# ViktorNfa/bluerov2_dynamics

Hardware: AMD Instinct MI355X
Metric: rk4_rollout_steps_per_s (higher is better)
Workload: dtype f64; 1 GPU; BASELINE config 2: 65536 trajectories/GPU x 5000 RK4 steps, thruster model, dt=0.02, iid U(-1,1) commands (splitmix64 stream 0x5EED), layout tpb, all states stored; trajectories_per_gpu=65536, horizon=5000, parallelism=1 x independent shards, no collective

## Files before the change

bluerov2_dynamics_amd/csrc/brov2_fast.h:

```cpp
#pragma once
#include "brov2_device.h"

namespace brov {

struct FastParams {
    double E[12];
    double da[6], db[6];
    double G[5];
    double lc[4][3];
    double ld[4];
    double Tm[6][8];
    double minv[6];
    double poly[5];
    double A1[9], b1[3];
    double A4[9], b4[3];
    double Ob[9];
    double al4[3];
    double Aw4[9], bw4[3];
    double g1[3];
    double XY[4];
    double cur[3];
    int has_current;
    int has_xy;
    int tm_dense;
// ... 8 lines not shown
    static constexpr bool RESIDENT = RES;
    double E[12], db[6];
    double da[6], G[5], ld[4], al4[3];
};
typedef HotConstsT<false> HotConsts;
typedef HotConstsT<true> HotConstsResident;

#ifndef BROV_CLAMP_BRANCH
#define BROV_CLAMP_BRANCH 1
#endif
#ifndef BROV_PSI_FRAME
#define BROV_PSI_FRAME 1
#endif
#define BROV_PIN_V(x) asm volatile("" : "+v"(x))
#define BROV_PIN_S(x) asm volatile("" : "+s"(x))
#define BROV_SC(h, p, f) (HC::RESIDENT ? (h).f : (p)->f)

template <bool RES>
__device__ __forceinline__ void load_hot(CFP pp, HotConstsT<RES>& h) {
    const auto& p = *pp;
#pragma unroll
    for (int i = 0; i < 12; ++i) { h.E[i] = p.E[i]; BROV_PIN_V(h.E[i]); }
#pragma unroll
    for (int i = 0; i < 6; ++i) { h.db[i] = p.db[i]; BROV_PIN_V(h.db[i]); }
    if constexpr (RES) {
#pragma unroll
        for (int i = 0; i < 6; ++i) { h.da[i] = p.da[i]; BROV_PIN_S(h.da[i]); }
#pragma unroll
        for (int i = 0; i < 5; ++i) { h.G[i] = p.G[i]; BROV_PIN_S(h.G[i]); }
#pragma unroll
        for (int i = 0; i < 4; ++i) { h.ld[i] = p.ld[i]; BROV_PIN_S(h.ld[i]); }
#pragma unroll
        for (int i = 0; i < 3; ++i) { h.al4[i] = p.al4[i]; BROV_PIN_S(h.al4[i]); }
    }
}

__device__ __forceinline__ CFP relaunder(CFP p) {
    asm volatile("" : "+s"(p));
    return p;
}

__device__ __forceinline__ void sincos_fast(double x, double& s, double& c, const double2* __restrict__ qt) {
    const double kf = rint(x * 6.36619772367581382433e-01);
    double r = fma(-kf, 1.57079632673412561417e+00, x);
    r = fma(-kf, 6.07710050630396597660e-11, r);
    r = fma(-kf, 2.02226624879595063154e-21, r);
    const int q = (int)kf;
    const double z = r * r;
    double ps = fma(z, 1.58969099521155010221e-10, -2.50507602534068634195e-08);
    ps = fma(z, ps, 2.75573137070700676789e-06);
    ps = fma(z, ps, -1.98412698298579493134e-04);
    ps = fma(z, ps, 8.33333333332248946124e-03);
    ps = fma(z, ps, -1.66666666666666324348e-01);
    const double sr = fma(z * r, ps, r);
    double pc = fma(z, -1.13596475577881948265e-11, 2.08757232129817482790e-09);
    pc = fma(z, pc, -2.75573143513906633035e-07);
    pc = fma(z, pc, 2.48015872894767294178e-05);
    pc = fma(z, pc, -1.38888888888741095749e-03);
    pc = fma(z, pc, 4.16666666666666019037e-02);
    const double cr = fma(z * z, pc, fma(-0.5, z, 1.0));
    const double2 t = qt[q & 3];
    s = fma(cr, t.y, sr * t.x);
    c = fma(-sr, t.y, cr * t.x);
}

__device__ __forceinline__ void init_quadrant_table(double2* qt) {
    if (threadIdx.x < 4) {
        const int q = threadIdx.x;
        qt[q] = make_double2(q == 0 ? 1.0 : (q == 2 ? -1.0 : 0.0), q == 1 ? 1.0 : (q == 3 ? -1.0 : 0.0));
    }
}

struct Trig { double sphi, cphi, sth, cth, spsi, cpsi; };

__device__ __forceinline__ void trig_full(const double* ang, Trig& t, const double2* __restrict__ qt) {
    sincos_fast(ang[0], t.sphi, t.cphi, qt);
    sincos_fast(ang[1], t.sth, t.cth, qt);
    sincos_fast(ang[2], t.spsi, t.cpsi, qt);
}

template <bool SHORT = false>
__device__ __forceinline__ void trig_delta(const Trig& b, const double d[3], Trig& t, double* dpsi = nullptr) {
    double dd[3] = {d[0], d[1], d[2]};
    int k = 0;
    const double m = fmax(fmax(fabs(d[0]), fabs(d[1])), fabs(d[2]));
    if (!(m <= (SHORT ? 0.0625 : 0.125))) {
        int e;
        (void)frexp(m, &e);
        k = e + (SHORT ? 4 : 3);
        double sc = ldexp(1.0, -k);
        if (!(m < 0x1p37)) { sc = __builtin_nan(""); k = 0; }
#pragma unroll
        for (int i = 0; i < 3; ++i) dd[i] *= sc;
    }
    double sd[3], cm[3];
#pragma unroll
    for (int i = 0; i < 3; ++i) {
        const double z = dd[i] * dd[i];
        double ps, pc;
        if constexpr (SHORT) {
            ps = fma(z, -1.98412698298579493134e-04, 8.33333333332248946124e-03);
            pc = fma(z, 2.48015872894767294178e-05, -1.38888888888741095749e-03);
        } else {
            ps = fma(z, 2.75573137070700676789e-06, -1.98412698298579493134e-04);
            ps = fma(z, ps, 8.33333333332248946124e-03);
            pc = fma(z, -2.75573143513906633035e-07, 2.48015872894767294178e-05);
            pc = fma(z, pc, -1.38888888888741095749e-03);
        }
        ps = fma(z, ps, -1.66666666666666324348e-01);
        sd[i] = fma(z * dd[i], ps, dd[i]);
        pc = fma(z, pc, 4.16666666666666019037e-02);
        pc = fma(z, pc, -0.5);
        cm[i] = z * pc;
    }
    for (int j = 0; j < k; ++j) {
#pragma unroll
        for (int i = 0; i < 3; ++i) {
            const double t2 = sd[i] + sd[i];
            const double s2 = fma(t2, cm[i], t2);
            cm[i] = -(t2 * sd[i]);
            sd[i] = s2;
        }
    }
    t.sphi = fma(b.cphi, sd[0], fma(b.sphi, cm[0], b.sphi)); t.cphi = fma(-b.sphi, sd[0], fma(b.cphi, cm[0], b.cphi));
    t.sth = fma(b.cth, sd[1], fma(b.sth, cm[1], b.sth));     t.cth = fma(-b.sth, sd[1], fma(b.cth, cm[1], b.cth));
    t.spsi = fma(b.cpsi, sd[2], fma(b.spsi, cm[2], b.spsi)); t.cpsi = fma(-b.spsi, sd[2], fma(b.cpsi, cm[2], b.cpsi));
    if (dpsi) { dpsi[0] = sd[2]; dpsi[1] = cm[2]; }
}

#ifndef BROV_TRIG_SHORT
#define BROV_TRIG_SHORT 1
#endif
__device__ __forceinline__ double recip_fast(double x) {
    double y = __builtin_amdgcn_rcp(x);
    double e = fma(-x, y, 1.0);
    y = fma(y, e, y);
    e = fma(-x, y, 1.0);
    return fma(y, e, y);
}

template <bool GENERIC, class HC>
__device__ __forceinline__ void nu_dot_fast(const HC& h, CFP p, const double R[9], const double nu[6],
                                            const double a[6], double sth, double ctsp, double ctcp, double out[6]) {
    const double u = nu[0], v = nu[1], w = nu[2], pp = nu[3], q = nu[4], r = nu[5];
    double nr0 = u, nr1 = v, nr2 = w;
    if (GENERIC && p->has_current) {
        nr0 -= fma(R[6], p->cur[2], fma(R[3], p->cur[1], R[0] * p->cur[0]));
        nr1 -= fma(R[7], p->cur[2], fma(R[4], p->cur[1], R[1] * p->cur[0]));
        nr2 -= fma(R[8], p->cur[2], fma(R[5], p->cur[1], R[2] * p->cur[0]));
    }
    double o0 = fma(-h.E[0], w * q, a[0]);  o0 = fma(h.E[1], v * r, o0);
    double o1 = fma(-h.E[2], u * r, a[1]);  o1 = fma(h.E[3], w * pp, o1);
    double o2 = fma(-h.E[4], v * pp, a[2]); o2 = fma(h.E[5], u * q, o2);
    double o3 = fma(-h.E[6], v * w, a[3]);  o3 = fma(-h.E[7], q * r, o3);
    double o4 = fma(-h.E[8], u * w, a[4]);  o4 = fma(-h.E[9], pp * r, o4);
    double o5 = fma(-h.E[10], u * v, a[5]); o5 = fma(-h.E[11], pp * q, o5);
    o0 = fma(-fma(h.db[0], fabs(nr0), BROV_SC(h, p, da[0])), nr0, o0);
    o1 = fma(-fma(h.db[1], fabs(nr1), BROV_SC(h, p, da[1])), nr1, o1);
    o2 = fma(-fma(h.db[2], fabs(nr2), BROV_SC(h, p, da[2])), nr2, o2);
    o3 = fma(-fma(h.db[3], fabs(pp), BROV_SC(h, p, da[3])), pp, o3);
    o4 = fma(-fma(h.db[4], fabs(q), BROV_SC(h, p, da[4])), q, o4);
    o5 = fma(-fma(h.db[5], fabs(r), BROV_SC(h, p, da[5])), r, o5);
    o0 = fma(-BROV_SC(h, p, G[0]), sth, o0);
    o1 = fma(BROV_SC(h, p, G[1]), ctsp, o1);
    o2 = fma(BROV_SC(h, p, G[2]), ctcp, o2);
    o3 = fma(BROV_SC(h, p, G[3]), ctsp, o3);
    o4 = fma(BROV_SC(h, p, G[4]), sth, o4);
    if (GENERIC && p->has_xy) {
        o3 = fma(-p->XY[0], ctcp, o3);
        o4 = fma(p->XY[1], ctcp, o4);
        o5 = fma(-p->XY[2], ctsp, o5);
        o5 = fma(-p->XY[3], sth, o5);
    }
    out[0] = o0; out[1] = o1; out[2] = o2; out[3] = o3; out[4] = o4; out[5] = o5;
}

template <bool GENERIC, class HC, bool PFRAME = false>
__device__ __forceinline__ void rhs_fast_euler(const HC& h, CFP p, const double x[12], const double a[6], double xd[12], const Trig& tg) {
    const double sphi = tg.sphi, cphi = tg.cphi, sth = tg.sth, cth = tg.cth, spsi = tg.spsi, cpsi = tg.cpsi;
    const double* nu = x + 6;
    const double ctsp = cth * sphi, ctcp = cth * cphi;
    if constexpr (GENERIC) {
        double R[9];
        const double ss = sth * sphi, sc = sth * cphi;
        R[0] = cpsi * cth; R[1] = fma(cpsi, ss, -(spsi * cphi)); R[2] = fma(cpsi, sc, spsi * sphi);
        R[3] = spsi * cth; R[4] = fma(spsi, ss, cpsi * cphi);    R[5] = fma(spsi, sc, -(cpsi * sphi));
        R[6] = -sth;       R[7] = ctsp;                          R[8] = ctcp;
        nu_dot_fast<true>(h, p, R, nu, a, sth, ctsp, ctcp, xd + 6);
#pragma unroll
        for (int i = 0; i < 3; ++i) xd[i] = fma(R[3 * i + 2], nu[2], fma(R[3 * i + 1], nu[1], R[3 * i] * nu[0]));
    } else {
        nu_dot_fast<false>(h, p, nullptr, nu, a, sth, ctsp, ctcp, xd + 6);
        const double y1 = fma(cphi, nu[1], -(sphi * nu[2])), z1 = fma(sphi, nu[1], cphi * nu[2]);
        const double x2 = fma(cth, nu[0], sth * z1), z2 = fma(cth, z1, -(sth * nu[0]));
        if constexpr (PFRAME) { xd[0] = x2; xd[1] = y1; }
        else {
            xd[0] = fma(cpsi, x2, -(spsi * y1));
            xd[1] = fma(spsi, x2, cpsi * y1);
        }
        xd[2] = z2;
    }
    double cc = cth;
#if BROV_CLAMP_BRANCH
    if (__builtin_amdgcn_ballot_w64(fabs(cc) < 1e-7) != 0) {
// ... 115 lines not shown
        }
    }
    __device__ __forceinline__ void obs_advance1(CFP p, const double acmd[6]) {
        const double c0 = p->al4[0], c1 = p->al4[1], c2 = p->al4[2], g0 = p->g1[0], g1 = p->g1[1], g2 = p->g1[2];
#pragma unroll
        for (int k = 0; k < 6; ++k) {
            const double a0 = z[k][0], a1 = z[k][1], a2 = z[k][2];
            z[k][0] = fma(g0, acmd[k], a1);
            z[k][1] = fma(g1, acmd[k], a2);
            z[k][2] = fma(c2, a2, fma(c1, a1, fma(c0, a0, g2 * acmd[k])));
        }
    }
    __device__ __forceinline__ void advance(const double __attribute__((address_space(4)))* A, const double __attribute__((address_space(4)))* b, const double acmd[6]) {
#pragma unroll
        for (int k = 0; k < 6; ++k) {
            const double a0 = z[k][0], a1 = z[k][1], a2 = z[k][2];
            const double q0 = fma(A[1], a1, fma(A[0], a0, b[0] * acmd[k]));
            const double q1 = fma(A[4], a1, fma(A[3], a0, b[1] * acmd[k]));
            const double q2 = fma(A[7], a1, fma(A[6], a0, b[2] * acmd[k]));
            double n0 = a0, n1 = a1, n2 = a2;
            asm("v_fma_f64 %0, %1, %2, %3" : "+v"(n0) : "s"(A[2]), "v"(a2), "v"(q0), "v"(q1), "v"(q2));
            asm("v_fma_f64 %0, %1, %2, %3" : "+v"(n1) : "s"(A[5]), "v"(a2), "v"(q1), "v"(q0), "v"(q2));
            asm("v_fma_f64 %0, %1, %0, %2" : "+v"(n2) : "s"(A[8]), "v"(q2), "v"(n0), "v"(n1));
            z[k][0] = n0; z[k][1] = n1; z[k][2] = n2;
        }
    }
};

__device__ __forceinline__ void advance_thrusters(const double __attribute__((address_space(4)))* A, const double __attribute__((address_space(4)))* b, const double fcmd[8], double X[8][3]) {
#pragma unroll
    for (int i = 0; i < 8; ++i) {
        const double a0 = X[i][0], a1 = X[i][1], a2 = X[i][2];
        X[i][0] = fma(A[2], a2, fma(A[1], a1, fma(A[0], a0, b[0] * fcmd[i])));
        X[i][1] = fma(A[5], a2, fma(A[4], a1, fma(A[3], a0, b[1] * fcmd[i])));
        X[i][2] = fma(A[8], a2, fma(A[7], a1, fma(A[6], a0, b[2] * fcmd[i])));
    }
}

template <int MODEL, bool SPARSE>
__device__ __forceinline__ void command_accel(CFP p, const double* u, double fcmd[8], double acmd[6]) {
    if constexpr (MODEL == MODEL_THRUSTER_EULER) {
#pragma unroll
        for (int i = 0; i < 8; ++i) {
            const double V = u[i], V2 = V * V;
            double hh = fma(V2, p->poly[4], p->poly[3]);
            hh = fma(V2, hh, p->poly[2]);
            hh = fma(V2, hh, p->poly[1]);
            hh = fma(V2, hh, p->poly[0]);
            fcmd[i] = V * hh;
        }
        if constexpr (SPARSE) {
#pragma unroll
            for (int k = 0; k < 6; ++k) {
                const int i0 = (k == 2) ? 4 : 0, i1 = (k == 3 || k == 4) ? 8 : (k == 2 ? 8 : 4);
                double a = p->Tm[k][i0] * fcmd[i0];
#pragma unroll
                for (int i = i0 + 1; i < i1; ++i) a = fma(p->Tm[k][i], fcmd[i], a);
                acmd[k] = a;
            }
        } else {
#pragma unroll
            for (int k = 0; k < 6; ++k) {
                double a = p->Tm[k][0] * fcmd[0];
#pragma unroll
                for (int i = 1; i < 8; ++i) a = fma(p->Tm[k][i], fcmd[i], a);
                acmd[k] = a;
            }
        }
    } else if constexpr (model_is_di(MODEL)) {
        constexpr int NU = Dims<MODEL>::NU;
#pragma unroll
        for (int k = 0; k < 6; ++k) {
            double a = p->Tm[k][0] * u[0];
#pragma unroll
            for (int i = 1; i < NU; ++i) a = fma(p->Tm[k][i], u[i], a);
            acmd[k] = a;
        }
    } else {
#pragma unroll
        for (int k = 0; k < 6; ++k) acmd[k] = p->minv[k] * u[k];
    }
}

template <int MODEL, int INTEG, bool GENERIC, class HC, class AccelFn>
__device__ __forceinline__ void integrate_fast(const HC& h, CFP p, double dt, double* x, AccelFn&& accel,
                                               const double2* qt, Trig* carry, bool refresh) {
    constexpr int NX = Dims<MODEL>::NX;
    constexpr bool ANG = !model_is_quat(MODEL);
    double a[6];
    Trig tb, ts;
    const bool CARRY = ANG && carry != nullptr;
    if constexpr (ANG) {
        if (!CARRY || refresh) trig_full(x + 3, tb, qt);
        else tb = *carry;
    }
    double dang[3];
    if constexpr (INTEG == INTEG_EULER) {
        double k[NX];
        accel(1, a);
        rhs_fast<MODEL, GENERIC>(h, p, x, a, k, tb);
        if (CARRY) {
#pragma unroll
            for (int i = 0; i < NX; ++i) {
                if (i >= 3 && i < 6) { dang[i - 3] = dt * k[i]; x[i] += dang[i - 3]; }
                else x[i] = fma(dt, k[i], x[i]);
            }
        } else {
#pragma unroll
            for (int i = 0; i < NX; ++i) x[i] = fma(dt, k[i], x[i]);
        }
    } else {
        double k[NX], xn[NX], xs[NX], dl[3];
        const double h2 = 0.5 * dt, h6 = dt / 6.0, h3 = dt / 3.0;
        constexpr bool PSIF = BROV_PSI_FRAME && ANG && !GENERIC && !model_is_di(MODEL);
        double dps[2] = {0.0, 0.0};
        auto stage_state = [&](double c, auto HALF) {
#pragma unroll
            for (int i = 0; i < NX; ++i) {
                if (ANG && i >= 3 && i < 6) dl[i - 3] = c * k[i];
                else xs[i] = fma(c, k[i], x[i]);
            }
            if constexpr (ANG) trig_delta<BROV_TRIG_SHORT && decltype(HALF)::value>(tb, dl, ts, PSIF ? dps : nullptr);
        };
        auto add_turned = [&](double w) {
            const double r0 = fma(dps[1], k[0], fma(-dps[0], k[1], k[0])), r1 = fma(dps[0], k[0], fma(dps[1], k[1], k[1]));
            xn[0] = fma(w, r0, xn[0]);
            xn[1] = fma(w, r1, xn[1]);
        };
        accel(1, a);
        rhs_fast<MODEL, GENERIC, HC, PSIF>(h, p, x, a, k, tb);
#pragma unroll
        for (int i = 0; i < NX; ++i) xn[i] = ((CARRY && i >= 3 && i < 6) || (PSIF && i < 2)) ? h6 * k[i] : fma(h6, k[i], x[i]);
        stage_state(h2, std::true_type{});
        accel(2, a);
        rhs_fast<MODEL, GENERIC, HC, PSIF>(h, p, xs, a, k, ts);
#pragma unroll
        for (int i = PSIF ? 2 : 0; i < NX; ++i) xn[i] = fma(h3, k[i], xn[i]);
        if constexpr (PSIF) add_turned(h3);
        stage_state(h2, std::true_type{});
        accel(3, a);
        rhs_fast<MODEL, GENERIC, HC, PSIF>(h, p, xs, a, k, ts);
#pragma unroll
        for (int i = PSIF ? 2 : 0; i < NX; ++i) xn[i] = fma(h3, k[i], xn[i]);
        if constexpr (PSIF) add_turned(h3);
        stage_state(dt, std::false_type{});
        accel(4, a);
        rhs_fast<MODEL, GENERIC, HC, PSIF>(h, p, xs, a, k, ts);
        if constexpr (PSIF) {
            add_turned(h6);
            x[0] = fma(tb.cpsi, xn[0], fma(-tb.spsi, xn[1], x[0]));
            x[1] = fma(tb.spsi, xn[0], fma(tb.cpsi, xn[1], x[1]));
        }
        if (CARRY) {
#pragma unroll
            for (int i = PSIF ? 2 : 0; i < NX; ++i) {
                if (i >= 3 && i < 6) { dang[i - 3] = fma(h6, k[i], xn[i]); x[i] += dang[i - 3]; }
                else x[i] = fma(h6, k[i], xn[i]);
            }
        } else {
#pragma unroll
            for (int i = PSIF ? 2 : 0; i < NX; ++i) x[i] = fma(h6, k[i], xn[i]);
        }
    }
    if constexpr (ANG) { if (CARRY) trig_delta(tb, dang, *carry); }
    if constexpr (model_is_quat(MODEL)) quat_normalize(x + 3);
}

template <int INTEG, int LAGMODE, bool TRACK, bool GENERIC>
__device__ __forceinline__ void lag_step_advance(CFP pl, LagZ& lz, const double fcmd[8], const double acmd[6], double X[8][3]) {
    constexpr bool OBS = !GENERIC;
    if constexpr (INTEG == INTEG_RK4 && LAGMODE == 0) {
        if constexpr (OBS) lz.advance(pl->Aw4, pl->bw4, acmd); else lz.advance(pl->A4, pl->b4, acmd);
        if constexpr (TRACK) advance_thrusters(pl->A4, pl->b4, fcmd, X);
    } else {
        if constexpr (OBS) lz.obs_advance1(pl, acmd); else lz.advance(pl->A1, pl->b1, acmd);
        if constexpr (TRACK) advance_thrusters(pl->A1, pl->b1, fcmd, X);
    }
}
template <int LAGMODE, bool GENERIC, class HC>
__device__ __forceinline__ void lag_stage_accel(const HC& h, CFP p, const LagZ& lz, int s, const double acmd[6], double a[6]) {
    const int se = LAGMODE == 0 ? s : 1;
    if constexpr (!GENERIC) lz.obs_accel_after(h, p, se, acmd, a); else lz.accel_after(p, se, acmd, a);
}

template <int MODEL, int INTEG, int LAGMODE, bool TRACK, bool GENERIC, class HC>
__device__ __forceinline__ void step_fast(const HC& h, CFP p0, double dt, double* x, const double* u,
                                          LagZ& lz, double X[8][3], const double2* qt, Trig* carry = nullptr, bool refresh = true) {
    constexpr bool THR = (MODEL == MODEL_THRUSTER_EULER);
    CFP p = relaunder(p0);
    double fcmd[8], acmd[6];
    if constexpr (MODEL == MODEL_DI_WRENCH_QUAT) quat_normalize(x + 3);
    command_accel<MODEL, !GENERIC>(p, u, fcmd, acmd);
    integrate_fast<MODEL, INTEG, GENERIC>(h, p, dt, x, [&](int s, double* a) {
        if constexpr (THR) lag_stage_accel<LAGMODE, GENERIC>(h, p, lz, s, acmd, a);
        else {
#pragma unroll
            for (int k = 0; k < 6; ++k) a[k] = acmd[k];
        }
    }, qt, carry, refresh);
    if constexpr (THR) lag_step_advance<INTEG, LAGMODE, TRACK, GENERIC>(relaunder(p0), lz, fcmd, acmd, X);
}

}
```

bluerov2_dynamics_amd/csrc/rollout.hip:

```cpp
#include "brov2_device.h"
#include "brov2_fast.h"
#include "brov2_kernels.h"

namespace brov {

constexpr int TRIG_REFRESH = 64;

#if BROV_CLOCK_STAMPS
__device__ unsigned long long g_clock_stamps[4096][4];
extern "C" __attribute__((visibility("default"))) int brov_debug_clock_stamps(unsigned long long* host, int nblocks) {
    return (int)hipMemcpyFromSymbol(host, HIP_SYMBOL(g_clock_stamps), sizeof(unsigned long long) * 4 * nblocks, 0, hipMemcpyDeviceToHost);
}
#endif

template <int N>
__device__ __forceinline__ void load_row(const double* __restrict__ src, double* r) {
    if constexpr (N % 2 == 0) {
        const double2* s2 = reinterpret_cast<const double2*>(src);
#pragma unroll
        for (int i = 0; i < N / 2; ++i) { double2 v = s2[i]; r[2 * i] = v.x; r[2 * i + 1] = v.y; }
    } else {
#pragma unroll
        for (int i = 0; i < N; ++i) r[i] = src[i];
    }
}
template <int N>
__device__ __forceinline__ void store_row(double* __restrict__ dst, const double* r) {
    if constexpr (N % 2 == 0) {
        double2* d2 = reinterpret_cast<double2*>(dst);
#pragma unroll
        for (int i = 0; i < N / 2; ++i) d2[i] = make_double2(r[2 * i], r[2 * i + 1]);
    } else {
#pragma unroll
        for (int i = 0; i < N; ++i) dst[i] = r[i];
    }
}
template <int N>
__device__ __forceinline__ void load_soa(const double* __restrict__ src, int64_t ld, double* r) {
#pragma unroll
    for (int i = 0; i < N; ++i) r[i] = src[i * ld];
}
template <int N>
__device__ __forceinline__ void store_soa(double* __restrict__ dst, int64_t ld, const double* r) {
#pragma unroll
    for (int i = 0; i < N; ++i) dst[i * ld] = r[i];
}
template <int N>
__device__ __forceinline__ void load_pairs(const double* __restrict__ p, int64_t ld2, double* r) {
#pragma unroll
    for (int i = 0; i < (N + 1) / 2; ++i) {
        typedef double v2d __attribute__((ext_vector_type(2)));
        const v2d w = __builtin_nontemporal_load(reinterpret_cast<const v2d*>(p + i * ld2));
        const double2 v = make_double2(w[0], w[1]);
        r[2 * i] = v.x;
        if (2 * i + 1 < N) r[2 * i + 1] = v.y;
    }
}
template <int N>
__device__ __forceinline__ void store_pairs(double* __restrict__ p, int64_t ld2, const double* r) {
#pragma unroll
    for (int i = 0; i < (N + 1) / 2; ++i) {
        typedef double v2d __attribute__((ext_vector_type(2)));
        v2d w; w[0] = r[2 * i]; w[1] = (2 * i + 1 < N) ? r[2 * i + 1] : 0.0;
        __builtin_nontemporal_store(w, reinterpret_cast<v2d*>(p + i * ld2));
    }
}

template <int MODEL, int INTEG, int LAGMODE>
__device__ __forceinline__ void integrate_step(const DevParams& p, double dt, double* x, const double* u, LagBank& lag) {
    constexpr int NX = Dims<MODEL>::NX;
    constexpr bool THR = (MODEL == MODEL_THRUSTER_EULER);
    double fcmd[8], F[8], tau[6];
    if constexpr (THR) {
#pragma unroll
        for (int i = 0; i < 8; ++i) fcmd[i] = thrust_poly(p, u[i]);
    } else {
#pragma unroll
        for (int i = 0; i < 6; ++i) tau[i] = u[i];
    }
    if constexpr (INTEG == INTEG_EULER) {
        double k[NX];
        if constexpr (THR) { lag.forces_after(p, 1, fcmd, F); allocate(p, F, tau); }
        rhs_state<MODEL>(p, x, tau, k);
#pragma unroll
        for (int i = 0; i < NX; ++i) x[i] = fma(dt, k[i], x[i]);
        if constexpr (THR) lag.advance(p, 1, fcmd);
    } else {
        double k[NX], acc[NX], xs[NX];
        const double h2 = 0.5 * dt;
        if constexpr (THR) { lag.forces_after(p, 1, fcmd, F); allocate(p, F, tau); }
        rhs_state<MODEL>(p, x, tau, k);
#pragma unroll
        for (int i = 0; i < NX; ++i) { acc[i] = k[i]; xs[i] = fma(h2, k[i], x[i]); }
        if constexpr (THR && LAGMODE == 0) { lag.forces_after(p, 2, fcmd, F); allocate(p, F, tau); }
// ... 84 lines not shown
    load_row<NX>(X0 + b * NX, x);
    LagZ lz;
    double Xl[8][3];
    if constexpr (MODEL == MODEL_THRUSTER_EULER) {
        if constexpr (TRACK) {
            load_row<24>(lag_io + b * 24, &Xl[0][0]);
            lz.from_thrusters(p, Xl);
        } else {
            lz.zero();
        }
        if constexpr (!GENERIC) lz.to_observer(p);
    }
    const int64_t rows = traj ? T / stride + 1 : 0;
    double* tp = nullptr;
    int64_t tstep = 0;
    constexpr int NXP = (NX + 1) / 2, NUP = (NU + 1) / 2;
    if (traj) {
        if constexpr (LAYOUT == LAYOUT_BTU) { tp = traj + b * rows * NX; tstep = NX; }
        else if constexpr (LAYOUT == LAYOUT_TUB) { tp = traj + b; tstep = (int64_t)NX * B; }
        else { tp = traj + 2 * b; tstep = (int64_t)NXP * 2 * B; }
    }
    auto store_state = [&]() {
        if constexpr (LAYOUT == LAYOUT_BTU) store_row<NX>(tp, x);
        else if constexpr (LAYOUT == LAYOUT_TUB) store_soa<NX>(tp, B, x);
        else store_pairs<NX>(tp, 2 * B, x);
        tp += tstep;
    };
    const double* up;
    int64_t ustep;
    if constexpr (LAYOUT == LAYOUT_BTU) { up = U + b * T * NU; ustep = NU; }
    else if constexpr (LAYOUT == LAYOUT_TUB) { up = U + b; ustep = (int64_t)NU * B; }
    else { up = U + 2 * b; ustep = (int64_t)NUP * 2 * B; }

    double un[NU];
    if (T > 0) {
        if constexpr (LAYOUT == LAYOUT_BTU) load_row<NU>(up, un);
        else if constexpr (LAYOUT == LAYOUT_TUB) load_soa<NU>(up, B, un);
        else load_pairs<NU>(up, 2 * B, un);
    }
    if (traj) store_state();
    int64_t countdown = stride;
    Trig tcarry;
#if BROV_CLOCK_STAMPS
    const unsigned long long st0 = __builtin_amdgcn_s_memtime(), sr0 = __builtin_amdgcn_s_memrealtime();
#endif
    for (int64_t t = 0; t < T; ++t) {
        double u[NU];
#pragma unroll
        for (int i = 0; i < NU; ++i) u[i] = un[i];
        up += (t + 1 < T) ? ustep : 0;
        {
            if constexpr (LAYOUT == LAYOUT_BTU) load_row<NU>(up, un);
            else if constexpr (LAYOUT == LAYOUT_TUB) load_soa<NU>(up, B, un);
            else load_pairs<NU>(up, 2 * B, un);
        }
        step_fast<MODEL, INTEG, LAGMODE, TRACK, GENERIC>(h, p, dt, x, u, lz, Xl, qt, &tcarry, (t & (TRIG_REFRESH - 1)) == 0);
        if (traj && --countdown == 0) {
            countdown = stride;
            store_state();
        }
    }
#if BROV_CLOCK_STAMPS
    if (threadIdx.x == 0 && blockIdx.x < 4096) {
        g_clock_stamps[blockIdx.x][0] = st0; g_clock_stamps[blockIdx.x][1] = sr0;
        g_clock_stamps[blockIdx.x][2] = __builtin_amdgcn_s_memtime(); g_clock_stamps[blockIdx.x][3] = __builtin_amdgcn_s_memrealtime();
    }
#endif
    if (XT) store_row<NX>(XT + b * NX, x);
    if constexpr (MODEL == MODEL_THRUSTER_EULER && TRACK) store_row<24>(lag_io + b * 24, &Xl[0][0]);
}

#ifndef BROV_PAIR_EXP
#define BROV_PAIR_EXP 0
#endif
#ifndef BROV_PAIR_RING
#define BROV_PAIR_RING 2
#endif
#ifndef BROV_PAIR_STAGE
#define BROV_PAIR_STAGE 1
#endif
#ifndef BROV_PAIR_PRIO
#define BROV_PAIR_PRIO 0
#endif
__device__ __forceinline__ void pair_barrier() { asm volatile("s_waitcnt lgkmcnt(0)\n\ts_barrier" ::: "memory"); }

__host__ __device__ constexpr bool pair_saddr_fits(int64_t B) { return B > 0 && B <= (int64_t)((0xFFFFFFFFull - 64 * 16) / (5 * 16)); }
__device__ __forceinline__ uint64_t lane_offset(unsigned& o) { asm volatile("" : "+v"(o)); return o; }
typedef __attribute__((address_space(1))) char* gptr_t;
__device__ __forceinline__ gptr_t wave_uniform(const void* ptr) {
    const uint64_t a = reinterpret_cast<uint64_t>(ptr);
    return (gptr_t)(((uint64_t)(unsigned)__builtin_amdgcn_readfirstlane((int)(a >> 32)) << 32) |
                    (uint64_t)(unsigned)__builtin_amdgcn_readfirstlane((int)(a & 0xFFFFFFFFull)));
}

template <int INTEG, int LAYOUT, int LAGMODE, bool TRACK, bool GENERIC>
__global__ void __launch_bounds__(512) rollout_pair_kernel(const FastParams* __restrict__ pg, int64_t B, int64_t T, double dt,
                                                           const double* __restrict__ X0, const double* __restrict__ U,
                                                           double* __restrict__ lag_io, double* __restrict__ traj,
                                                           int64_t stride, double* __restrict__ XT) {
    constexpr int MODEL = MODEL_THRUSTER_EULER;
    constexpr int NX = 12, NU = 8, NXP = 6, NUP = 4;
    constexpr int NS = (INTEG == INTEG_RK4) ? 4 : 1;
    __shared__ double2 qt[4];
    __shared__ __attribute__((aligned(16))) double2 xch[BROV_PAIR_RING][4][NS * 3][64];
    constexpr bool STG = (LAYOUT == LAYOUT_BTU) && BROV_PAIR_STAGE;
    constexpr int STG_S = 2, STG_ROW = STG_S * NXP + 1, STG_PER = STG_S * NXP;
    __shared__ __attribute__((aligned(16))) double2 stg[STG ? 4 * 64 * STG_ROW : 1];
#if BROV_PAIR_EXP == 4
    __shared__ int pflag[2][4];
    if (threadIdx.x < 8) (&pflag[0][0])[threadIdx.x] = 0;
#endif
    init_quadrant_table(qt);
    __syncthreads();
    const int wave = threadIdx.x >> 6, pair = wave & 3, lane = threadIdx.x & 63;
    const bool thrust = wave >= 4;
#if BROV_PAIR_PRIO
    if (thrust) __builtin_amdgcn_s_setprio(0); else __builtin_amdgcn_s_setprio(3);
#endif
    const int64_t b_raw = (int64_t)blockIdx.x * 256 + pair * 64 + lane;
    const bool live = b_raw < B;
    const int64_t b = live ? b_raw : B - 1;
    const CFP p = as_constant(pg);
    HotConstsResident h;
    load_hot(p, h);

    if (thrust) {
        LagZ lz;
        double Xl[8][3];
        if constexpr (TRACK) { load_row<24>(lag_io + b * 24, &Xl[0][0]); lz.from_thrusters(p, Xl); }
        else lz.zero();
        if constexpr (!GENERIC) lz.to_observer(p);
        const double* up = nullptr;
        int64_t ustep;
        if constexpr (LAYOUT == LAYOUT_BTU) { up = U + b * T * NU; ustep = NU; }
        else if constexpr (LAYOUT == LAYOUT_TUB) { up = U + b; ustep = (int64_t)NU * B; }
        else ustep = (int64_t)NUP * 2 * B;
        const int64_t bw_c = (int64_t)blockIdx.x * 256 + pair * 64 < B ? (int64_t)blockIdx.x * 256 + pair * 64 : B - 1;
        gptr_t ub = LAYOUT == LAYOUT_TPB ? wave_uniform(U + 2 * bw_c) : nullptr;
        unsigned uoff[NUP];
#pragma unroll
        for (int i = 0; i < NUP; ++i) uoff[i] = (unsigned)((b - bw_c) * 16 + (int64_t)i * 16 * B);
        double un[NU];
        int64_t tl = 0;
        auto load_controls = [&]() {
            if constexpr (LAYOUT == LAYOUT_BTU) load_row<NU>(up, un);
            else if constexpr (LAYOUT == LAYOUT_TUB) load_soa<NU>(up, B, un);
            else {
                typedef double v2d __attribute__((ext_vector_type(2)));
#pragma unroll
                for (int i = 0; i < NUP; ++i) {
                    const v2d w = __builtin_nontemporal_load(reinterpret_cast<const __attribute__((address_space(1))) v2d*>(ub + lane_offset(uoff[i])));
                    un[2 * i] = w[0]; un[2 * i + 1] = w[1];
                }
            }
        };
        if (T > 0) load_controls();
        auto produce = [&](int slot) {
            double fcmd[8], acmd[6], a[6];
            const CFP pp = relaunder(p);
            command_accel<MODEL, !GENERIC>(pp, un, fcmd, acmd);
            if constexpr (LAYOUT == LAYOUT_TPB) ub += (tl + 1 != T) ? ustep * 8 : 0;
            else up += (tl + 1 != T) ? ustep : 0;
            ++tl;
            load_controls();
#pragma unroll
            for (int s = 1; s <= NS; ++s) {
                lag_stage_accel<LAGMODE, GENERIC>(h, pp, lz, s, acmd, a);
#pragma unroll
                for (int j = 0; j < 3; ++j) xch[slot][pair][(s - 1) * 3 + j][lane] = make_double2(a[2 * j], a[2 * j + 1]);
            }
            lag_step_advance<INTEG, LAGMODE, TRACK, GENERIC>(relaunder(p), lz, fcmd, acmd, Xl);
        };
#if BROV_PAIR_EXP == 1
        for (int64_t t = 0; t < T; ++t) pair_barrier();
        (void)produce;
#elif BROV_PAIR_EXP == 4
        {
            volatile int* prodf = &pflag[0][pair];
            volatile int* consf = &pflag[1][pair];
            int slot = 0;
            for (int64_t s = 0; s < T; ++s) {
                if (s >= BROV_PAIR_RING) {
                    const int need = (int)(s - BROV_PAIR_RING + 1);
                    int spins = 0;
                    while (*consf < need && ++spins < (1 << 22)) __builtin_amdgcn_s_sleep(1);
                }
                asm volatile("" ::: "memory");
                produce(slot);
                asm volatile("" ::: "memory");
                *prodf = (int)(s + 1);
                slot = (slot + 1 == BROV_PAIR_RING) ? 0 : slot + 1;
            }
        }
#else
        if (T > 0) produce(0);
        for (int64_t t = 1; t < T; ++t) {
            pair_barrier();
            produce((int)(t & 1));
        }
        if (T > 0) pair_barrier();
#endif
        if constexpr (TRACK) { if (live) store_row<24>(lag_io + b * 24, &Xl[0][0]); }
    } else {
        double x[NX];
        load_row<NX>(X0 + b * NX, x);
        double* tp = nullptr;
        int64_t tstep = 0;
        if (traj) {
            if constexpr (LAYOUT == LAYOUT_BTU) { tp = traj + b * (T / stride + 1) * NX; tstep = NX; }
            else if constexpr (LAYOUT == LAYOUT_TUB) { tp = traj + b; tstep = (int64_t)NX * B; }
            else tstep = (int64_t)NXP * 2 * B;
        }
        const int64_t sw_c = (int64_t)blockIdx.x * 256 + pair * 64 < B ? (int64_t)blockIdx.x * 256 + pair * 64 : B - 1;
        gptr_t sb = LAYOUT == LAYOUT_TPB ? wave_uniform(traj + 2 * sw_c) : nullptr;
        unsigned soff[NXP];
#pragma unroll
        for (int i = 0; i < NXP; ++i) soff[i] = (unsigned)((b - sw_c) * 16 + (int64_t)i * 16 * B);
        const bool staged = STG && traj != nullptr && stride == 1 && (uint64_t)(T + 1) * (NX * 8) * 64 < (1ull << 32);
        const int64_t bw = (int64_t)blockIdx.x * 256 + pair * 64;
        constexpr int STG_TPI = 64 / STG_PER, STG_NI = (64 + STG_TPI - 1) / STG_TPI;
        const int st_q = lane / STG_PER, st_c = lane - st_q * STG_PER;
        const unsigned st_rb = (unsigned)((T + 1) * (NX * 8));
        const unsigned st_off = (unsigned)st_q * st_rb + (unsigned)st_c * 16u;
        const int st_lds = st_q * STG_ROW + st_c;
        const int st_live = (int)((B - bw) < 64 ? (B - bw) : 64);
        int st_fill = 0;
        char* st_base = nullptr;
        double2* const st_wave = stg + (STG ? pair * 64 * STG_ROW : 0);
        if constexpr (STG) {
            if (staged) {
                const uint64_t a = reinterpret_cast<uint64_t>(traj) + (uint64_t)bw * (uint64_t)st_rb;
                st_base = reinterpret_cast<char*>(((uint64_t)(unsigned)__builtin_amdgcn_readfirstlane((int)(a >> 32)) << 32) |
                                                  (uint64_t)(unsigned)__builtin_amdgcn_readfirstlane((int)(a & 0xFFFFFFFFull)));
            }
        }
        auto st_flush = [&](int ns) {
            if constexpr (STG) {
                __builtin_amdgcn_wave_barrier();
                asm volatile("s_waitcnt lgkmcnt(0)" ::: "memory");
                if (ns == STG_S) {
#pragma unroll
                    for (int it = 0; it < STG_NI; ++it) {
                        if (lane < STG_TPI * STG_PER && it * STG_TPI + st_q < st_live) {
                            const double2 v = st_wave[st_lds + it * STG_TPI * STG_ROW];
                            *reinterpret_cast<double2*>(st_base + (uint64_t)(it * STG_TPI) * st_rb + st_off) = v;
                        }
                    }
                } else {
                    const int per = ns * NXP;
                    for (int i = lane; i < 64 * per; i += 64) {
                        const int q = i / per, c = i - q * per;
                        const double2 v = st_wave[q * STG_ROW + c];
                        if (q < st_live) *reinterpret_cast<double2*>(st_base + (uint64_t)q * st_rb + (uint64_t)c * 16u) = v;
                    }
                }
                st_base += (int64_t)ns * (NX * 8);
                st_fill = 0;
                __builtin_amdgcn_wave_barrier();
                asm volatile("s_waitcnt lgkmcnt(0)" ::: "memory");
            }
        };
        auto store_state = [&]() {
            if constexpr (STG) {
                if (staged) {
                    double2* row = st_wave + lane * STG_ROW + st_fill * NXP;
#pragma unroll
                    for (int j = 0; j < NXP; ++j) row[j] = make_double2(x[2 * j], x[2 * j + 1]);
                    if (++st_fill == STG_S) st_flush(STG_S);
                    return;
                }
            }
            if constexpr (LAYOUT == LAYOUT_TPB) {
                typedef double v2d __attribute__((ext_vector_type(2)));
#pragma unroll
                for (int i = 0; i < NXP; ++i) {
                    v2d w; w[0] = x[2 * i]; w[1] = x[2 * i + 1];
                    __builtin_nontemporal_store(w, reinterpret_cast<__attribute__((address_space(1))) v2d*>(sb + lane_offset(soff[i])));
                }
                sb += tstep * 8;
                return;
            }
            if (live) {
                if constexpr (LAYOUT == LAYOUT_BTU) store_row<NX>(tp, x);
                else if constexpr (LAYOUT == LAYOUT_TUB) store_soa<NX>(tp, B, x);
            }
            tp += tstep;
        };
        if (traj) store_state();
        int64_t countdown = stride;
        Trig tcarry;
#if BROV_CLOCK_STAMPS
        const unsigned long long st0 = __builtin_amdgcn_s_memtime(), sr0 = __builtin_amdgcn_s_memrealtime();
#endif
#if BROV_PAIR_EXP == 4
        volatile int* prodf = &pflag[0][pair];
        volatile int* consf = &pflag[1][pair];
        int seen = 0, slot = 0;
#endif
        for (int64_t t = 0; t < T; ++t) {
#if BROV_PAIR_EXP == 3
            pair_barrier();
            const double2* src = &xch[t & 1][pair][0][lane];
            if (T >= 0) continue;
#elif BROV_PAIR_EXP == 4
            {
                int spins = 0;
                while (seen < (int)(t + 1) && ++spins < (1 << 22)) { seen = *prodf; if (seen < (int)(t + 1)) __builtin_amdgcn_s_sleep(1); }
            }
            asm volatile("" ::: "memory");
            const double2* src = &xch[slot][pair][0][lane];
            slot = (slot + 1 == BROV_PAIR_RING) ? 0 : slot + 1;
#else
            pair_barrier();
            const double2* src = &xch[t & 1][pair][0][lane];
#endif
            integrate_fast<MODEL, INTEG, GENERIC>(h, p, dt, x, [&](int s, double* a) {
#pragma unroll
                for (int j = 0; j < 3; ++j) { const double2 v = src[((s - 1) * 3 + j) * 64]; a[2 * j] = v.x; a[2 * j + 1] = v.y; }
            }, qt, &tcarry, (t & (TRIG_REFRESH - 1)) == 0);
#if BROV_PAIR_EXP == 4
            asm volatile("" ::: "memory");
            *consf = (int)(t + 1);
            seen = *prodf;
#endif
            if (traj && --countdown == 0) {
                countdown = stride;
                store_state();
            }
        }
#if BROV_CLOCK_STAMPS
        if (wave == 0 && lane == 0 && blockIdx.x < 4096) {
            g_clock_stamps[blockIdx.x][0] = st0; g_clock_stamps[blockIdx.x][1] = sr0;
            g_clock_stamps[blockIdx.x][2] = __builtin_amdgcn_s_memtime(); g_clock_stamps[blockIdx.x][3] = __builtin_amdgcn_s_memrealtime();
        }
#endif
        if constexpr (STG) { if (staged && st_fill > 0) st_flush(st_fill); }
        if (XT && live) store_row<NX>(XT + b * NX, x);
    }
}

constexpr int BTU_TILE = 2;

template <int NU> __device__ __forceinline__ int in_swizzle(int d, int j) {
    if constexpr (NU == 8) return d ^ ((j >> 1) & 7);
    else return d;
}

template <int MODEL, int INTEG, int LAGMODE, bool TRACK, bool GENERIC>
__global__ void __launch_bounds__(256) rollout_btu_lds_kernel(const FastParams* __restrict__ pg, int64_t B, int64_t T, double dt,
                                                              const double* __restrict__ X0, const double* __restrict__ U,
                                                              double* __restrict__ lag_io, double* __restrict__ traj,
                                                              double* __restrict__ XT) {
    constexpr int NX = Dims<MODEL>::NX, NU = Dims<MODEL>::NU;
    constexpr int CH = BTU_TILE * NU / 2;
    constexpr int IN_SLOTS = 64 * CH;
    constexpr int ORS = BTU_TILE * NX + 2;
    constexpr int OCB = (NX % 2 == 0) ? 2 : 1;
    constexpr int OCPR = BTU_TILE * NX / OCB;
    __shared__ __attribute__((aligned(16))) double lds_in[4][2][IN_SLOTS * 2];
    __shared__ __attribute__((aligned(16))) double lds_out[4][64 * ORS];
    __shared__ double2 qt[4];
    init_quadrant_table(qt);
    __syncthreads();

    const int lane = threadIdx.x & 63, wave = threadIdx.x >> 6;
    const int64_t b0w = (int64_t)blockIdx.x * 256 + wave * 64;
    const int64_t b_raw = b0w + lane;
    const bool live = b_raw < B;
    const int64_t b = live ? b_raw : B - 1;
    const CFP p = as_constant(pg);
    HotConsts h;
    load_hot(p, h);
    double x[NX];
    load_row<NX>(X0 + b * NX, x);
    LagZ lz;
    double Xl[8][3];
    if constexpr (MODEL == MODEL_THRUSTER_EULER) {
        if constexpr (TRACK) { load_row<24>(lag_io + b * 24, &Xl[0][0]); lz.from_thrusters(p, Xl); }
        else lz.zero();
        if constexpr (!GENERIC) lz.to_observer(p);
    }
    if (traj && live) store_row<NX>(traj + b * (T + 1) * NX, x);

    auto issue_tile = [&](int64_t k) {
        const int64_t t0 = k * BTU_TILE;
#pragma unroll
        for (int i = 0; i < CH; ++i) {
            const int g = i * 64 + lane;
            const int j = g / CH, c = g % CH;
            const int d = in_swizzle<NU>(c, j);
            int64_t bj = b0w + j;
            if (bj >= B) bj = B - 1;
            int64_t t = t0 + (2 * d) / NU;
            if (t >= T) t = T - 1;
            const double* src = U + (bj * T + t) * NU + (2 * d) % NU;
            __builtin_amdgcn_global_load_lds((const __attribute__((address_space(1))) void*)src,
                                             (__attribute__((address_space(3))) void*)(&lds_in[wave][k & 1][i * 128]), 16, 0, 0);
        }
    };

    const int64_t ntiles = (T + BTU_TILE - 1) / BTU_TILE;
    Trig tcarry;
    if (ntiles > 0) issue_tile(0);
    for (int64_t k = 0; k < ntiles; ++k) {
        __syncthreads();
        if (k + 1 < ntiles) issue_tile(k + 1);
        const double* ib = &lds_in[wave][k & 1][0];
        double* ob = &lds_out[wave][lane * ORS];
        const int64_t t0 = k * BTU_TILE;
#pragma unroll 1
        for (int s = 0; s < BTU_TILE; ++s) {
            if (t0 + s < T) {
// ... 299 lines not shown
```

Measured before the change: 29.11 billion steps/s.

## Prefetch next-stage RK4 commands early and make trig range extension wave-uniform

The consumer wave now loads each RK4 stage's command inputs from LDS one stage ahead, using a second register buffer, so LDS latency overlaps the previous rhs evaluation. trig_delta's range-extension and doubling loops are gated by a wave-wide ballot, giving a uniform branch that skips the rare path entirely. The pair barrier is rewritten with builtins and a specific waitcnt mask. Optional phase-timing instrumentation is added behind a compile flag. The extra live registers could lower occupancy.

```diff
diff --git a/bluerov2_dynamics_amd/csrc/brov2_fast.h b/bluerov2_dynamics_amd/csrc/brov2_fast.h
--- a/bluerov2_dynamics_amd/csrc/brov2_fast.h
+++ b/bluerov2_dynamics_amd/csrc/brov2_fast.h
@@ -114,16 +114,22 @@
 template <bool SHORT = false>
 __device__ __forceinline__ void trig_delta(const Trig& b, const double d[3], Trig& t, double* dpsi = nullptr) {
     double dd[3] = {d[0], d[1], d[2]};
-    int k = 0;
+    int k;
     const double m = fmax(fmax(fabs(d[0]), fabs(d[1])), fabs(d[2]));
-    if (!(m <= (SHORT ? 0.0625 : 0.125))) {
-        int e;
-        (void)frexp(m, &e);
-        k = e + (SHORT ? 4 : 3);
-        double sc = ldexp(1.0, -k);
-        if (!(m < 0x1p37)) { sc = __builtin_nan(""); k = 0; }
-#pragma unroll
-        for (int i = 0; i < 3; ++i) dd[i] *= sc;
+    const bool far = !(m <= (SHORT ? 0.0625 : 0.125));
+    const bool any_far = __builtin_amdgcn_ballot_w64(far) != 0;
+    if (any_far) {
+        asm volatile("; trig_delta range extension, rare" ::: "memory");
+        k = 0;
+        if (far) {
+            int e;
+            (void)frexp(m, &e);
+            k = e + (SHORT ? 4 : 3);
+            double sc = ldexp(1.0, -k);
+            if (!(m < 0x1p37)) { sc = __builtin_nan(""); k = 0; }
+#pragma unroll
+            for (int i = 0; i < 3; ++i) dd[i] *= sc;
+        }
     }
     double sd[3], cm[3];
 #pragma unroll
@@ -145,13 +151,16 @@
         pc = fma(z, pc, -0.5);
         cm[i] = z * pc;
     }
-    for (int j = 0; j < k; ++j) {
-#pragma unroll
-        for (int i = 0; i < 3; ++i) {
-            const double t2 = sd[i] + sd[i];
-            const double s2 = fma(t2, cm[i], t2);
-            cm[i] = -(t2 * sd[i]);
-            sd[i] = s2;
+    if (any_far) {
+        asm volatile("; trig_delta doubling, rare" ::: "memory");
+        for (int j = 0; j < k; ++j) {
+#pragma unroll
+            for (int i = 0; i < 3; ++i) {
+                const double t2 = sd[i] + sd[i];
+                const double s2 = fma(t2, cm[i], t2);
+                cm[i] = -(t2 * sd[i]);
+                sd[i] = s2;
+            }
         }
     }
     t.sphi = fma(b.cphi, sd[0], fma(b.sphi, cm[0], b.sphi)); t.cphi = fma(-b.sphi, sd[0], fma(b.cphi, cm[0], b.cphi));
@@ -433,12 +442,12 @@
     }
 }
 
-template <int MODEL, int INTEG, bool GENERIC, class HC, class AccelFn>
+template <int MODEL, int INTEG, bool GENERIC, bool AHEAD = false, class HC, class AccelFn>
 __device__ __forceinline__ void integrate_fast(const HC& h, CFP p, double dt, double* x, AccelFn&& accel,
                                                const double2* qt, Trig* carry, bool refresh) {
     constexpr int NX = Dims<MODEL>::NX;
     constexpr bool ANG = !model_is_quat(MODEL);
-    double a[6];
+    double a[6], an[6];
     Trig tb, ts;
     const bool CARRY = ANG && carry != nullptr;
     if constexpr (ANG) {
@@ -479,24 +488,26 @@
             xn[1] = fma(w, r1, xn[1]);
         };
         accel(1, a);
+        if constexpr (AHEAD) accel(2, an);
         rhs_fast<MODEL, GENERIC, HC, PSIF>(h, p, x, a, k, tb);
 #pragma unroll
         for (int i = 0; i < NX; ++i) xn[i] = ((CARRY && i >= 3 && i < 6) || (PSIF && i < 2)) ? h6 * k[i] : fma(h6, k[i], x[i]);
         stage_state(h2, std::true_type{});
-        accel(2, a);
-        rhs_fast<MODEL, GENERIC, HC, PSIF>(h, p, xs, a, k, ts);
+        if constexpr (AHEAD) { accel(3, a); rhs_fast<MODEL, GENERIC, HC, PSIF>(h, p, xs, an, k, ts); }
+        else { accel(2, a); rhs_fast<MODEL, GENERIC, HC, PSIF>(h, p, xs, a, k, ts); }
 #pragma unroll
         for (int i = PSIF ? 2 : 0; i < NX; ++i) xn[i] = fma(h3, k[i], xn[i]);
         if constexpr (PSIF) add_turned(h3);
         stage_state(h2, std::true_type{});
-        accel(3, a);
+        if constexpr (AHEAD) accel(4, an);
+        else accel(3, a);
         rhs_fast<MODEL, GENERIC, HC, PSIF>(h, p, xs, a, k, ts);
 #pragma unroll
         for (int i = PSIF ? 2 : 0; i < NX; ++i) xn[i] = fma(h3, k[i], xn[i]);
         if constexpr (PSIF) add_turned(h3);
         stage_state(dt, std::false_type{});
-        accel(4, a);
-        rhs_fast<MODEL, GENERIC, HC, PSIF>(h, p, xs, a, k, ts);
+        if constexpr (AHEAD) rhs_fast<MODEL, GENERIC, HC, PSIF>(h, p, xs, an, k, ts);
+        else { accel(4, a); rhs_fast<MODEL, GENERIC, HC, PSIF>(h, p, xs, a, k, ts); }
         if constexpr (PSIF) {
             add_turned(h6);
             x[0] = fma(tb.cpsi, xn[0], fma(-tb.spsi, xn[1], x[0]));
diff --git a/bluerov2_dynamics_amd/csrc/rollout.hip b/bluerov2_dynamics_amd/csrc/rollout.hip
--- a/bluerov2_dynamics_amd/csrc/rollout.hip
+++ b/bluerov2_dynamics_amd/csrc/rollout.hip
@@ -10,6 +10,18 @@
 __device__ unsigned long long g_clock_stamps[4096][4];
 extern "C" __attribute__((visibility("default"))) int brov_debug_clock_stamps(unsigned long long* host, int nblocks) {
     return (int)hipMemcpyFromSymbol(host, HIP_SYMBOL(g_clock_stamps), sizeof(unsigned long long) * 4 * nblocks, 0, hipMemcpyDeviceToHost);
+}
+#endif
+
+#if BROV_PHASE_STAMPS
+__device__ unsigned long long g_phase_stamps[4096][8];
+extern "C" __attribute__((visibility("default"))) int brov_debug_phase_stamps(unsigned long long* host, int nblocks) {
+    return (int)hipMemcpyFromSymbol(host, HIP_SYMBOL(g_phase_stamps), sizeof(unsigned long long) * 8 * nblocks, 0, hipMemcpyDeviceToHost);
+}
+__device__ __forceinline__ unsigned long long phase_stamp() {
+    unsigned long long t;
+    asm volatile("s_memtime %0\n\ts_waitcnt lgkmcnt(0)" : "=s"(t) :: "memory");
+    return t;
 }
 #endif
 
@@ -260,7 +272,12 @@
 #ifndef BROV_PAIR_PRIO
 #define BROV_PAIR_PRIO 0
 #endif
-__device__ __forceinline__ void pair_barrier() { asm volatile("s_waitcnt lgkmcnt(0)\n\ts_barrier" ::: "memory"); }
+__device__ __forceinline__ void pair_barrier() {
+    asm volatile("" ::: "memory");
+    __builtin_amdgcn_s_waitcnt(0xC07F);
+    __builtin_amdgcn_s_barrier();
+    asm volatile("" ::: "memory");
+}
 
 __host__ __device__ constexpr bool pair_saddr_fits(int64_t B) { return B > 0 && B <= (int64_t)((0xFFFFFFFFull - 64 * 16) / (5 * 16)); }
 __device__ __forceinline__ uint64_t lane_offset(unsigned& o) { asm volatile("" : "+v"(o)); return o; }
@@ -371,12 +388,27 @@
             }
         }
 #else
+#if BROV_PHASE_STAMPS
+        unsigned long long ph_wait = 0, ph_prod = 0;
+        if (T > 0) produce(0);
+        for (int64_t t = 1; t < T; ++t) {
+            const unsigned long long ta = phase_stamp();
+            pair_barrier();
+            const unsigned long long tr = phase_stamp();
+            produce((int)(t & 1));
+            const unsigned long long td = phase_stamp();
+            ph_wait += tr - ta; ph_prod += td - tr;
+        }
+        if (T > 0) pair_barrier();
+        if (pair == 0 && lane == 0 && blockIdx.x < 4096) { g_phase_stamps[blockIdx.x][3] = ph_wait; g_phase_stamps[blockIdx.x][4] = ph_prod; }
+#else
         if (T > 0) produce(0);
         for (int64_t t = 1; t < T; ++t) {
             pair_barrier();
             produce((int)(t & 1));
         }
         if (T > 0) pair_barrier();
+#endif
 #endif
         if constexpr (TRACK) { if (live) store_row<24>(lag_io + b * 24, &Xl[0][0]); }
     } else {
@@ -475,7 +507,15 @@
         volatile int* consf = &pflag[1][pair];
         int seen = 0, slot = 0;
 #endif
+#if BROV_PHASE_STAMPS
+        unsigned long long ph_wait = 0, ph_comp = 0, ph_store = 0, ph_prev = 0;
+        const unsigned long long ph_t0 = __builtin_amdgcn_s_memtime(), ph_r0 = __builtin_amdgcn_s_memrealtime();
+#endif
         for (int64_t t = 0; t < T; ++t) {
+#if BROV_PHASE_STAMPS
+            const unsigned long long ta = phase_stamp();
+            if (t > 0) ph_store += ta - ph_prev;
+#endif
 #if BROV_PAIR_EXP == 3
             pair_barrier();
             const double2* src = &xch[t & 1][pair][0][lane];
@@ -492,10 +532,20 @@
             pair_barrier();
             const double2* src = &xch[t & 1][pair][0][lane];
 #endif
-            integrate_fast<MODEL, INTEG, GENERIC>(h, p, dt, x, [&](int s, double* a) {
+#if BROV_PHASE_STAMPS
+            const unsigned long long tr = phase_stamp();
+            ph_wait += tr - ta;
+#endif
+            integrate_fast<MODEL, INTEG, GENERIC, true>(h, p, dt, x, [&](int s, double* a) {
 #pragma unroll
                 for (int j = 0; j < 3; ++j) { const double2 v = src[((s - 1) * 3 + j) * 64]; a[2 * j] = v.x; a[2 * j + 1] = v.y; }
             }, qt, &tcarry, (t & (TRIG_REFRESH - 1)) == 0);
+#if BROV_PHASE_STAMPS
+#pragma unroll
+            for (int i = 0; i < NX; ++i) asm volatile("" :: "v"(x[i]));
+            ph_prev = phase_stamp();
+            ph_comp += ph_prev - tr;
+#endif
 #if BROV_PAIR_EXP == 4
             asm volatile("" ::: "memory");
             *consf = (int)(t + 1);
@@ -506,6 +556,15 @@
                 store_state();
             }
         }
+#if BROV_PHASE_STAMPS
+        if (pair == 0 && lane == 0 && blockIdx.x < 4096) {
+            const unsigned long long ph_t1 = __builtin_amdgcn_s_memtime(), ph_r1 = __builtin_amdgcn_s_memrealtime();
+            if (T > 0) ph_store += ph_t1 - ph_prev;
+            g_phase_stamps[blockIdx.x][0] = ph_wait; g_phase_stamps[blockIdx.x][1] = ph_comp; g_phase_stamps[blockIdx.x][2] = ph_store;
+            g_phase_stamps[blockIdx.x][5] = (unsigned long long)T;
+            g_phase_stamps[blockIdx.x][6] = ph_t1 - ph_t0; g_phase_stamps[blockIdx.x][7] = ph_r1 - ph_r0;
+        }
+#endif
 #if BROV_CLOCK_STAMPS
         if (wave == 0 && lane == 0 && blockIdx.x < 4096) {
             g_clock_stamps[blockIdx.x][0] = st0; g_clock_stamps[blockIdx.x][1] = sr0;
```

New measurement: 29.21 billion steps/s, median of 6. About the same (+0.3%).
